# xinntao/EDVR

Hardware: AMD Instinct MI355X
Metric: EDVR-L x4 5-frame 720p clips/sec (higher is better)
Workload: dtype fp32 emulated as 2xf16 (hi+lo, 22-bit operands, 4 cross products), fp32 accumulate; 1 GPU; EDVR-L x4, 5 frames, 180x320 LR -> 720x1280, batch 10/GPU, inference; clips_per_gpu=10, global_clips=10, parallelism=clip-sharded x1, no data-path collective, world_size=1, backend=single process

## Files before the change

edvr_amd/_lib.py:

```python
import ctypes
import os

_HERE = os.path.dirname(os.path.abspath(__file__))
LIB_PATH = os.environ.get('EDVR_AMD_LIB') or os.path.join(_HERE, 'lib', 'libedvr_amd.so')

c_float_p = ctypes.c_void_p
i32, i64, f32, sz = ctypes.c_int, ctypes.c_int64, ctypes.c_float, ctypes.c_size_t
vp = ctypes.c_void_p


class ConvDesc(ctypes.Structure):
    _fields_ = [
        ('x1', vp), ('x2', vp), ('c1', i32), ('c2', i32), ('x1_img_stride', i64), ('x2_img_stride', i64),
        ('x2_div', i32), ('x2_mul', i32), ('x2_add', i32), ('n', i32), ('h', i32), ('w', i32), ('wpk', vp),
        ('bias', vp), ('co', i32), ('ks', i32), ('stride', i32), ('act', i32), ('act_from', i32), ('res1', vp),
        ('res2', vp), ('res1_img_stride', i64), ('res2_img_stride', i64), ('y', vp), ('y_img_stride', i64),
        ('out_mode', i32), ('algo', i32), ('gate', vp), ('gate_img_stride', i64), ('gate_slope', f32), ('y_scale', f32),
        ('wpk_f4', vp), ('abs_sum', vp), ('abs_sum_channels', i32), ('wpk_f4s', vp), ('x_amax', vp), ('y_amax', vp),
        ('pre', vp), ('pre_img_stride', i64), ('pre_div', i32), ('pre_mul', i32), ('pre_add', i32), ('pre_n', i32),
    ]


PROTOTYPES = {
    'edvr_version': (ctypes.c_char_p, []),
# ... 54 lines not shown
    'edvr_bd_downsample_u8': (i32, [vp, vp, i32, i32, i32, i32, i32, i32, i32, vp]),
    'edvr_bd_downsample_f32': (i32, [vp, vp, i32, i32, i32, i64, i32, i32, i32, i32, vp]),
    'edvr_imresize_bicubic_u8_windows': (i32, [vp, vp, vp, vp, i32, i32, i32, i32, i32, i32, vp]),
    'edvr_bd_downsample_u8_windows': (i32, [vp, vp, vp, vp, i32, i32, i32, i32, i32, i32, vp]),
    'edvr_adam_chunk_bytes': (sz, []),
    'edvr_adam_multi_f32': (i32, [vp, i32, ctypes.c_float, ctypes.c_float, ctypes.c_float, vp]),
    'edvr_dcnv1_fwd_ws_bytes': (sz, [i32] * 12),
    'edvr_dcnv1_fwd_f32': (i32, [vp] * 4 + [i32] * 12 + [i64, i32, vp, sz, vp]),
    'edvr_dcnv1_bwd_ws_bytes': (sz, [i32] * 12),
    'edvr_dcnv1_bwd_f32': (i32, [vp] * 7 + [i32] * 12 + [i64, i64, i32, vp, sz, vp]),
    'edvr_dcnv2_bwd_f32': (i32, [vp] * 10 + [i32] * 12 + [i64, i64, i64, i64, i32, vp, sz, vp]),
    'edvr_dcnv2_bwd_split_f32': (i32, [vp] * 10 + [i32] * 12 + [i64, i64, i64, i64, i32, vp, sz, vp, vp, vp]),
    'edvr_dcnv2_bwd_split_applies': (i32, []),
    'edvr_tsa_temporal_f32': (i32, [vp] * 5 + [i32] * 4 + [vp]),
    'edvr_tsa_temporal_pair_f32': (i32, [vp] * 5 + [i32] * 4 + [vp]),
    'edvr_pool_maxavg_3x3s2_f32': (i32, [vp, vp, i32, i32, i32, i32, vp]),
    'edvr_upsample2x_f32': (i32, [vp, vp, i32, i32, i32, f32, vp]),
    'edvr_tsa_combine_f32': (i32, [vp, vp, vp, vp, i64, vp]),
    'edvr_upsample4x_add_f32': (i32, [vp, vp, i32, i32, i32, vp]),
    'edvr_add_f32': (i32, [vp, vp, vp, i64, vp]),
    'edvr_act_bwd_f32': (i32, [vp, vp, vp, vp, vp, i32, i32, i64, i32, i32, vp]),
    'edvr_conv2d_wgrad_ws_bytes': (sz, [i32] * 7),
    'edvr_conv2d_wgrad_algo': (i32, [i32]),
    'edvr_conv2d_wgrad_kernel_name': (i32, [i32] * 8 + [ctypes.c_char_p, sz]),
    'edvr_conv2d_wgrad_f32': (i32, [vp] * 4 + [i32] * 8 + [i64, i64, i32, i32, i32, i64, i32, vp, vp, sz, vp]),
    'edvr_conv2d_wgrad_split_f32': (i32, [vp] * 4 + [i32] * 8 + [i64, i64, i32, i32, i32, i64, i32, vp, vp, sz, vp, vp, vp]),
    'edvr_conv2d_wgrad_split_applies': (i32, [i32] * 8),
    'edvr_conv2d_wgrad_split_is_direct': (i32, [i32] * 2),
    'edvr_channel_sum_f32': (i32, [vp, vp, i32, i32, i64, i64, vp, sz, vp]),
    'edvr_pixel_unshuffle2_f32': (i32, [vp, vp, i32, i32, i32, i32, vp]),
# ... 45 lines not shown
```

edvr_amd/csrc/conv1x1_s.hip:

```cpp
#include <cstdlib>

#include "common.h"
#include "pack.h"

namespace edvr {

typedef float f32x16 __attribute__((ext_vector_type(16)));
typedef int c1s_i32x4 __attribute__((ext_vector_type(4)));
typedef _Float16 c1s_f16x8 __attribute__((ext_vector_type(8)));

namespace {
__device__ __forceinline__ void c1s_split4(const float (&x)[4], float s, unsigned (&o)[4]) {
  asm volatile(
      "v_fma_mixlo_f16 %0, %4, %8, 0\n\tv_fma_mixlo_f16 %1, %5, %8, 0\n\tv_fma_mixlo_f16 %2, %6, %8, 0\n\tv_fma_mixlo_f16 %3, %7, %8, 0\n\t"
      "v_fma_mixhi_f16 %0, %4, %8, -%0 op_sel_hi:[0,0,1]\n\tv_fma_mixhi_f16 %1, %5, %8, -%1 op_sel_hi:[0,0,1]\n\t"
      "v_fma_mixhi_f16 %2, %6, %8, -%2 op_sel_hi:[0,0,1]\n\tv_fma_mixhi_f16 %3, %7, %8, -%3 op_sel_hi:[0,0,1]"
      : "=&v"(o[0]), "=&v"(o[1]), "=&v"(o[2]), "=&v"(o[3])
      : "v"(x[0]), "v"(x[1]), "v"(x[2]), "v"(x[3]), "s"(s));
}
__device__ __forceinline__ float c1s_scale(float amax) {
  const int be = (int)((__builtin_bit_cast(unsigned, amax) >> 23) & 255u);
  return __builtin_bit_cast(float, (unsigned)min(max(127 + 14 - (be - 127), 7), 215) << 23);
}
}

struct Conv1x1SArgs {
  edvr_conv2d_desc d;
  const unsigned *wq;
  int ci, cop, co_start;
  int seg_shift;
};

template <int MT>
__global__ __launch_bounds__(256, 2) void conv1x1_split_kernel(const Conv1x1SArgs a) {
  constexpr int CK = 64, MB = 32 * MT, DEPTH = 8, NW = CK * MB / 4 / 256;
  constexpr int RSRC_FLAGS = 0x00020000;
  constexpr int OOB = (int)0x80000000;
  __shared__ __attribute__((aligned(16))) unsigned wsm[2][CK * MB];
  const edvr_conv2d_desc &d = a.d;
  const float s_x = c1s_scale(__builtin_bit_cast(float, __builtin_amdgcn_readfirstlane(__builtin_bit_cast(int, *d.x_amax))));
  const float inv_sw = __builtin_bit_cast(float, __builtin_amdgcn_readfirstlane((int)a.wq[1]));
  const int tid = threadIdx.x, lane = tid & 63, half = lane >> 5, j = lane & 31;
  const int wave = __builtin_amdgcn_readfirstlane(tid >> 6);
  const int hw = d.h * d.w;
  const int img = blockIdx.z, co_blk = a.co_start + blockIdx.y * MB;
  const int p = (blockIdx.x * 4 + wave) * 32 + j;
  const bool p_ok = p < hw;

  auto uniform_ptr = [&](const float *ptr) {
    const uint64_t pv = reinterpret_cast<uint64_t>(ptr);
    return ((uint64_t)(uint32_t)__builtin_amdgcn_readfirstlane((int)(pv >> 32)) << 32) | (uint32_t)__builtin_amdgcn_readfirstlane((int)(uint32_t)pv);
  };
  const uint64_t b1 = uniform_ptr(d.x1 + (int64_t)img * d.x1_img_stride);
  uint64_t b2 = b1;
  if (d.x2) {
    const int i2 = d.x2_div > 0 ? (img / d.x2_div) * d.x2_mul + d.x2_add : img;
    b2 = uniform_ptr(d.x2 + (int64_t)i2 * d.x2_img_stride);
  }
  const int voff = p_ok ? (4 * half * hw + p) * 4 : OOB;
  const int real_steps = (d.c1 + d.c2) / 8;
  const int seg_mask = (1 << a.seg_shift) - 1;
  const int64_t plane_bytes = (int64_t)hw * 4;
  auto load_b = [&](int s, float (&v)[4]) {
    const int c = 8 * s;
    const bool first = c < d.c1;
    const int cc = first ? c : c - d.c1;
    const uint64_t base = (first ? b1 : b2) + (uint64_t)((int64_t)(cc & ~seg_mask) * plane_bytes);
    const __amdgpu_buffer_rsrc_t rs = __builtin_amdgcn_make_buffer_rsrc(reinterpret_cast<void *>(base), (short)0, 0x7fffffff, RSRC_FLAGS);
    const bool ok = s < real_steps;
#pragma unroll
    for (int i = 0; i < 4; ++i)
      v[i] = __builtin_bit_cast(float, __builtin_amdgcn_raw_buffer_load_b32(rs, ok ? voff : OOB, ok ? ((cc & seg_mask) + i) * hw * 4 : 0, 0));
  };

  const int quads_total = (d.c1 + d.c2 + 3) / 4;
  c1s_i32x4 wr[NW];
  auto w_load = [&](int c0) {
#pragma unroll
    for (int i = 0; i < NW; ++i) {
      const int e = tid + i * 256, q = e / MB, col = e - q * MB;
      const bool ok = c0 / 4 + q < quads_total;
      const c1s_i32x4 v = *reinterpret_cast<const c1s_i32x4 *>(a.wq + 16 + ((int64_t)(ok ? c0 / 4 + q : 0) * a.cop + co_blk + col) * 4);
      wr[i] = ok ? v : c1s_i32x4{0, 0, 0, 0};
    }
  };
  auto w_commit = [&](int buf) {
#pragma unroll
    for (int i = 0; i < NW; ++i) *reinterpret_cast<c1s_i32x4 *>(&wsm[buf][(tid + i * 256) * 4]) = wr[i];
  };
// ... 10 lines not shown
  w_commit(0);
  __syncthreads();

  const int chunks = a.ci / CK;
  for (int ch = 0; ch < chunks; ++ch) {
    const int buf = ch & 1;
    const bool more = ch + 1 < chunks;
    if (more) w_load((ch + 1) * CK);
    const unsigned *ws = wsm[buf] + (half * MB + j) * 4;
#pragma unroll
    for (int s = 0; s < CK / 8; ++s) {
      c1s_i32x4 av[MT];
#pragma unroll
      for (int m = 0; m < MT; ++m) av[m] = *reinterpret_cast<const c1s_i32x4 *>(ws + ((2 * s) * MB + m * 32) * 4);
      unsigned pk[4];
      c1s_split4(bq[s % DEPTH], s_x, pk);
      load_b(ch * (CK / 8) + s + DEPTH, bq[s % DEPTH]);
      c1s_i32x4 b, br;
#pragma unroll
      for (int q = 0; q < 4; ++q) {
        b[q] = (int)pk[q];
        br[q] = (int)__builtin_amdgcn_alignbit(pk[q], pk[q], 16);
      }
#pragma unroll
      for (int m = 0; m < MT; ++m) acc[m] = __builtin_amdgcn_mfma_f32_32x32x16_f16(__builtin_bit_cast(c1s_f16x8, av[m]), __builtin_bit_cast(c1s_f16x8, b), acc[m], 0, 0, 0);
#pragma unroll
      for (int m = 0; m < MT; ++m) acc[m] = __builtin_amdgcn_mfma_f32_32x32x16_f16(__builtin_bit_cast(c1s_f16x8, av[m]), __builtin_bit_cast(c1s_f16x8, br), acc[m], 0, 0, 0);
      if (s == CK / 16 && more) w_commit(buf ^ 1);
    }
    asm volatile("s_waitcnt lgkmcnt(0)\n\ts_barrier" ::: "memory");
// ... 16 lines not shown
          float v = __builtin_fmaf(acc[m][r], unscale, d.bias ? d.bias[co] : 0.f);
          if (co >= d.act_from) v = sig ? __builtin_amdgcn_rcpf(1.f + __expf(-v)) : fmaxf(v, slope * v);
          const int64_t off = (int64_t)co * hw + p;
          if (q1) v += q1[off];
          if (q2) v += q2[off];
          y[off] = v;
          vmax = max(vmax, __builtin_bit_cast(unsigned, v) & 0x7fffffffu);
        }
      }
  }
  if (d.y_amax) {
#pragma unroll
    for (int sh = 32; sh > 0; sh >>= 1) vmax = max(vmax, (unsigned)__shfl_xor((int)vmax, sh));
    if (lane == 0) atomicMax(reinterpret_cast<unsigned *>(d.y_amax), vmax);
  }
}

__global__ __launch_bounds__(1024) void conv1x1_split_scale_kernel(const float *__restrict__ w, unsigned *__restrict__ wq, int64_t total) {
  __shared__ float red[16];
  float m = 0.f;
  for (int64_t i = threadIdx.x; i < total; i += 1024) m = fmaxf(m, fabsf(w[i]));
#pragma unroll
  for (int sh = 32; sh > 0; sh >>= 1) m = fmaxf(m, __shfl_xor(m, sh));
  if ((threadIdx.x & 63) == 0) red[threadIdx.x >> 6] = m;
  __syncthreads();
  if (threadIdx.x == 0) {
    for (int i = 1; i < 16; ++i) m = fmaxf(m, red[i]);
    const unsigned field = f4s_weight_scale_field(__builtin_bit_cast(unsigned, m));
    wq[0] = field << 23;
    wq[1] = (254u - field) << 23;
// ... 43 lines not shown
  const int full = d.co / 128, rem_tiles = cdiv(d.co - full * 128, 32);
  if (full > 0) {
    a.co_start = 0;
    hipLaunchKernelGGL((conv1x1_split_kernel<4>), dim3(cdiv(hw, 128), full, d.n), dim3(256), 0, stream, a);
  }
  if (rem_tiles > 0) {
    a.co_start = full * 128;
    const dim3 grid(cdiv(hw, 128), 1, d.n);
    if (rem_tiles == 1) hipLaunchKernelGGL((conv1x1_split_kernel<1>), grid, dim3(256), 0, stream, a);
    else if (rem_tiles == 2) hipLaunchKernelGGL((conv1x1_split_kernel<2>), grid, dim3(256), 0, stream, a);
    else hipLaunchKernelGGL((conv1x1_split_kernel<3>), grid, dim3(256), 0, stream, a);
  }
  return check_launch("conv1x1_split_kernel");
}

}

extern "C" {

size_t edvr_conv2d_packed_weight_1x1s_elems(int co, int ci) {
  if (co <= 0 || ci <= 0) return 0;
  return 16 + (size_t)((ci + 63) / 64 * 16) * ((co + 127) / 128 * 128) * 4;
}

int edvr_conv2d_pack_weight_1x1s_f32(const float *w, void *wpk, int co, int ci, edvr_stream_t stream_) {
  using namespace edvr;
  EDVR_REQUIRE(w && wpk && co > 0 && ci > 0, "pack_weight_1x1s: bad arguments");
  EDVR_REQUIRE((reinterpret_cast<uintptr_t>(wpk) & 15) == 0, "pack_weight_1x1s: wpk must be 16-byte aligned");
  hipStream_t stream = as_stream(stream_);
  unsigned *wq = static_cast<unsigned *>(wpk);
  const int cop = (co + 127) / 128 * 128, quads = (ci + 63) / 64 * 16;
  hipLaunchKernelGGL(conv1x1_split_scale_kernel, dim3(1), dim3(1024), 0, stream, w, wq, (int64_t)co * ci);
  const int64_t total = (int64_t)quads * cop;
// ... 6 lines not shown
```

edvr_amd/csrc/elementwise.hip:

```cpp
#include "common.h"
#include "pixel.h"

namespace edvr {

__device__ __forceinline__ float sigmoidf(float v) { return 1.f / (1.f + __expf(-v)); }

template <int VEC, bool PAIR>
__device__ __forceinline__ void tsa_temporal_body(const float *__restrict__ emb, const float *__restrict__ emb_ref,
                                                  const float *__restrict__ aligned, float *__restrict__ out, float *__restrict__ out_rev,
                                                  float *__restrict__ prob_out, int b, int t, int c, int hw) {
  typedef float vec_t __attribute__((ext_vector_type(VEC)));
  const int hwv = hw / VEC;
  const int64_t total = (int64_t)b * t * hwv;
  for (int64_t idx = (int64_t)blockIdx.x * 256 + threadIdx.x; idx < total; idx += (int64_t)gridDim.x * 256) {
    const int pv = (int)(idx % hwv);
    const int ti = (int)((idx / hwv) % t);
    const int bi = (int)(idx / ((int64_t)hwv * t));
    const vec_t *e = reinterpret_cast<const vec_t *>(emb + ((int64_t)(bi * t + ti) * c) * hw) + pv;
    const vec_t *r = reinterpret_cast<const vec_t *>(emb_ref + ((int64_t)bi * c) * hw) + pv;
    vec_t dot = 0.f;
    for (int ch = 0; ch < c; ++ch) dot += e[(int64_t)ch * hwv] * r[(int64_t)ch * hwv];
    vec_t pr;
#pragma unroll
    for (int v = 0; v < VEC; ++v) pr[v] = sigmoidf(dot[v]);
    if (prob_out) reinterpret_cast<vec_t *>(prob_out + (int64_t)(bi * t + ti) * hw)[pv] = pr;
    const vec_t *a = reinterpret_cast<const vec_t *>(aligned + ((int64_t)(bi * t + ti) * c) * hw) + pv;
    vec_t *o = reinterpret_cast<vec_t *>(out + ((int64_t)(bi * t + ti) * c) * hw) + pv;
    if constexpr (PAIR) {
      vec_t *o2 = reinterpret_cast<vec_t *>(out_rev + ((int64_t)(bi * t + (t - 1 - ti)) * c) * hw) + pv;
      for (int ch = 0; ch < c; ++ch) {
        const vec_t m = a[(int64_t)ch * hwv] * pr;
        o[(int64_t)ch * hwv] = m;
        o2[(int64_t)ch * hwv] = m;
      }
    } else {
      for (int ch = 0; ch < c; ++ch) o[(int64_t)ch * hwv] = a[(int64_t)ch * hwv] * pr;
    }
  }
}

template <int VEC>
__global__ __launch_bounds__(256) void tsa_temporal_kernel(const float *__restrict__ emb, const float *__restrict__ emb_ref,
                                                           const float *__restrict__ aligned, float *__restrict__ out,
                                                           float *__restrict__ prob_out, int b, int t, int c, int hw) {
  tsa_temporal_body<VEC, false>(emb, emb_ref, aligned, out, nullptr, prob_out, b, t, c, hw);
}

template <int VEC>
__global__ __launch_bounds__(256) void tsa_temporal_pair_kernel(const float *__restrict__ emb, const float *__restrict__ emb_ref,
                                                                const float *__restrict__ aligned, float *__restrict__ out,
                                                                float *__restrict__ out_rev, int b, int t, int c, int hw) {
  tsa_temporal_body<VEC, true>(emb, emb_ref, aligned, out, out_rev, nullptr, b, t, c, hw);
}

__global__ __launch_bounds__(256) void pool_maxavg_kernel(const float *__restrict__ x, float *__restrict__ y, int n, int c, int h, int w,
                                                          int ho, int wo) {
  const int64_t total = (int64_t)n * c * ho * wo;
  for (int64_t idx = (int64_t)blockIdx.x * 256 + threadIdx.x; idx < total; idx += (int64_t)gridDim.x * 256) {
    const int ox = (int)(idx % wo);
    const int oy = (int)((idx / wo) % ho);
    const int ch = (int)((idx / ((int64_t)wo * ho)) % c);
    const int ni = (int)(idx / ((int64_t)wo * ho * c));
    const float *src = x + ((int64_t)ni * c + ch) * h * w;
    float mx = -INFINITY, sm = 0.f;
#pragma unroll
    for (int dy = 0; dy < 3; ++dy) {
      const int iy = oy * 2 - 1 + dy;
// ... 224 lines not shown

int edvr_tsa_temporal_f32(const float *emb, const float *emb_ref, const float *aligned, float *out, float *prob_out, int b, int t,
                          int c, int hw, edvr_stream_t stream) {
  using namespace edvr;
  EDVR_REQUIRE(emb && emb_ref && aligned && out && b > 0 && t > 0 && c > 0 && hw > 0, "tsa_temporal: bad arguments");
  if (hw % 4 == 0) {
    hipLaunchKernelGGL(tsa_temporal_kernel<4>, dim3(grid_for((int64_t)b * t * (hw / 4))), dim3(256), 0, as_stream(stream), emb, emb_ref,
                       aligned, out, prob_out, b, t, c, hw);
  } else {
    hipLaunchKernelGGL(tsa_temporal_kernel<1>, dim3(grid_for((int64_t)b * t * hw)), dim3(256), 0, as_stream(stream), emb, emb_ref,
                       aligned, out, prob_out, b, t, c, hw);
  }
  return check_launch("tsa_temporal_kernel");
}

int edvr_tsa_temporal_pair_f32(const float *emb, const float *emb_ref, const float *aligned, float *out, float *out_rev, int b, int t,
                               int c, int hw, edvr_stream_t stream) {
  using namespace edvr;
  EDVR_REQUIRE(emb && emb_ref && aligned && out && out_rev && b > 0 && t > 0 && c > 0 && hw > 0, "tsa_temporal_pair: bad arguments");
  const int64_t n = (int64_t)b * t * c * hw;
  EDVR_REQUIRE((out + n <= out_rev || out_rev + n <= out) && (out + n <= aligned || aligned + n <= out) &&
                   (out_rev + n <= aligned || aligned + n <= out_rev),
               "tsa_temporal_pair: out, out_rev and aligned must be distinct buffers");
  if (hw % 4 == 0) {
    hipLaunchKernelGGL(tsa_temporal_pair_kernel<4>, dim3(grid_for((int64_t)b * t * (hw / 4))), dim3(256), 0, as_stream(stream), emb,
                       emb_ref, aligned, out, out_rev, b, t, c, hw);
  } else {
    hipLaunchKernelGGL(tsa_temporal_pair_kernel<1>, dim3(grid_for((int64_t)b * t * hw)), dim3(256), 0, as_stream(stream), emb, emb_ref,
                       aligned, out, out_rev, b, t, c, hw);
  }
// ... 92 lines not shown
```

edvr_amd/edvr_arch.py:

```python
import torch
from torch import nn

from . import functional as F_
from .arch_util import DCNv2Pack, ResidualBlockNoBN, make_layer, warn_offset_absmean

LRELU = F_.ACT_LRELU


def _conv3(cin, cout, stride=1):
    return nn.Conv2d(cin, cout, 3, stride, 1)


class PCDAlignment(nn.Module):

    def __init__(self, num_feat=64, deformable_groups=8):
        super().__init__()
        self.offset_conv1, self.offset_conv2, self.offset_conv3 = nn.ModuleDict(), nn.ModuleDict(), nn.ModuleDict()
        self.dcn_pack, self.feat_conv = nn.ModuleDict(), nn.ModuleDict()
        for lv in (3, 2, 1):
            key = f'l{lv}'
            self.offset_conv1[key] = _conv3(2 * num_feat, num_feat)
            if lv == 3:
                self.offset_conv2[key] = _conv3(num_feat, num_feat)
            else:
# ... 47 lines not shown
        self.avg_pool = nn.AvgPool2d(3, stride=2, padding=1)
        self.spatial_attn1 = nn.Conv2d(num_frame * num_feat, num_feat, 1)
        self.spatial_attn2 = nn.Conv2d(num_feat * 2, num_feat, 1)
        self.spatial_attn3 = _conv3(num_feat, num_feat)
        self.spatial_attn4 = nn.Conv2d(num_feat, num_feat, 1)
        self.spatial_attn5 = _conv3(num_feat, num_feat)
        self.spatial_attn_l1 = nn.Conv2d(num_feat, num_feat, 1)
        self.spatial_attn_l2 = _conv3(num_feat * 2, num_feat)
        self.spatial_attn_l3 = _conv3(num_feat, num_feat)
        self.spatial_attn_add1 = nn.Conv2d(num_feat, num_feat, 1)
        self.spatial_attn_add2 = nn.Conv2d(num_feat, num_feat, 1)
        self.lrelu = nn.LeakyReLU(negative_slope=0.1, inplace=True)
        self.upsample = nn.Upsample(scale_factor=2, mode='bilinear', align_corners=False)

    def forward(self, aligned_feat):
        return self.spatial(self.temporal(aligned_feat))

    def temporal(self, aligned_feat, pair=False):
        b, t, c, h, w = aligned_feat.shape
        alias = F_.ops.carry_bound
        emb_ref = F_.conv(self.temporal_attn1, alias(aligned_feat[:, self.center_frame_idx], aligned_feat))
        emb = F_.conv(self.temporal_attn2, alias(aligned_feat.reshape(b * t, c, h, w), aligned_feat)).view(b, t, -1, h, w)
        if pair:
            mod, mod_rev = F_.tsa_temporal_pair(emb, emb_ref, aligned_feat)
            return alias(mod.view(b, t * c, h, w), mod), alias(mod_rev.view(b, t * c, h, w), mod_rev)
        mod = F_.tsa_temporal(emb, emb_ref, aligned_feat)
        return alias(mod.view(b, t * c, h, w), mod)

    def spatial(self, mod):
        feat = F_.conv(self.feat_fusion, mod, act=LRELU)
        attn = F_.conv(self.spatial_attn1, mod, act=LRELU)
        attn = F_.conv(self.spatial_attn2, F_.pool_maxavg(attn), act=LRELU)
        lvl = F_.conv(self.spatial_attn_l1, attn, act=LRELU)
        lvl = F_.conv(self.spatial_attn_l2, F_.pool_maxavg(lvl), act=LRELU)
        lvl = F_.upsample2x(F_.conv(self.spatial_attn_l3, lvl, act=LRELU))
        attn = F_.conv(self.spatial_attn3, attn, act=LRELU, res1=lvl)
        attn = F_.upsample2x(F_.conv(self.spatial_attn4, attn, act=LRELU))
        attn = F_.conv(self.spatial_attn5, attn)
        attn_add = F_.conv(self.spatial_attn_add2, F_.conv(self.spatial_attn_add1, attn, act=LRELU))
        return F_.tsa_combine(feat, attn, attn_add)


class PredeblurModule(nn.Module):

    def __init__(self, num_in_ch=3, num_feat=64, hr_in=False):
        super().__init__()
# ... 107 lines not shown
            f1 = F_.conv(self.conv_1x1, self.predeblur(frames), out=head)
        else:
            f1 = F_.conv(self.conv_first, frames, act=LRELU, out=head)
        if out is None:
            f1 = self.feature_extraction(f1)
        else:
            for i, blk in enumerate(blocks):
                f1 = blk(f1, out=o1 if i == len(blocks) - 1 else None)
        f2 = F_.conv(self.conv_l2_2, F_.conv(self.conv_l2_1, f1, act=LRELU), act=LRELU, out=o2)
        f3 = F_.conv(self.conv_l3_2, F_.conv(self.conv_l3_1, f2, act=LRELU), act=LRELU, out=o3)
        return [f1, f2, f3]

    def restore_from_features(self, pyr, x_center, b, t, out_dtype=torch.float32, out=None, keep=None, elem=None, accumulate='only', scale=1.0,
                              acc=None, bands=None):
        self._check_tail_args(out_dtype, out, keep, elem, accumulate, scale, acc, bands)
        operand, sink = self.align_windows(pyr, b, t)
        return self._restore_aligned(operand, x_center, b, t, out_dtype, out, keep, elem, accumulate, scale, acc, bands, sink)

    def align_windows(self, pyr, b, t, pair=False):
        f1, f2, f3 = pyr
        ctr = self.center_frame_idx
        h, w = f1.shape[2], f1.shape[3]
        if pair and 2 * ctr != t - 1:
            raise ValueError(f'align_windows(pair=True): the reversed clip keeps its centre only when it is the middle frame, got {ctr} of {t}')
        sink = []
        dcns = self.pcd_align.dcn_modules()
        for m in dcns:
            m.stats_sink = sink
        try:
            aligned = self.pcd_align.align([f1, f2, f3], [f1, f2, f3], ref_map=(t, t, ctr))
        finally:
            for m in dcns:
                m.stats_sink = None
        flat = aligned
        aligned = F_.ops.carry_bound(aligned.view(b, t, -1, h, w), aligned)
        if self.taps is not None:
            self.taps['aligned'] = aligned
        if self.with_tsa:
            operand = self.fusion.temporal(aligned, pair=pair)
            return (*operand, sink) if pair else (operand, sink)
        operand = F_.ops.carry_bound(aligned.view(b, -1, h, w), aligned)
        if not pair:
            return operand, sink
        if torch.is_grad_enabled():
            raise RuntimeError('align_windows(pair=True) has no backward: call it under torch.no_grad()')
        table = torch.arange(b * t, dtype=torch.int32, device=flat.device).view(b, t).flip(1).reshape(-1)
        rev = F_.ops.gather_images([flat], table)[0]
        return operand, F_.ops.carry_bound(rev.view(b, -1, h, w), rev), sink

    def restore_from_aligned(self, operand, x_center, b, t, out_dtype=torch.float32, out=None, keep=None, elem=None, accumulate='only', scale=1.0,
                             acc=None, bands=None, sink=None):
        self._check_tail_args(out_dtype, out, keep, elem, accumulate, scale, acc, bands)
        return self._restore_aligned(operand, x_center, b, t, out_dtype, out, keep, elem, accumulate, scale, acc, bands, sink)
# ... 4 lines not shown
            raise ValueError(f'out_dtype must be torch.float32 or torch.uint8, got {out_dtype}')
        if out_dtype == torch.uint8 and torch.is_grad_enabled():
            raise RuntimeError('the uint8 output of EDVR.restore_from_features has no backward: call it under torch.no_grad()')
        if out is None and keep is not None:
            raise ValueError('keep= names a rectangle of the result to store into out=: it needs out')
        if out is not None and torch.is_grad_enabled():
            raise RuntimeError('EDVR.restore_from_features(out=) writes in place and has no backward: call it under torch.no_grad()')
        if elem is None and (accumulate != 'only' or scale != 1.0 or (acc is not None and bands is None)):
            raise ValueError('accumulate=, scale= and acc= belong to a self-ensemble element: they need elem')
        if (elem is not None or bands is not None) and (out is None or (out_dtype == torch.uint8) != (acc is not None)):
            raise ValueError('elem= and bands= store into out= (and, with uint8 output, accumulate in acc=)')

    def _restore_aligned(self, operand, x_center, b, t, out_dtype, out, keep, elem, accumulate, scale, acc, bands, sink):
        dst = out
        taps = self.taps
        feat = self.fusion.spatial(operand) if self.with_tsa else F_.conv(self.fusion, operand)
        if taps is not None:
            taps['fused'] = feat
        out = self.reconstruction(feat)
        if taps is not None:
            taps['trunk'] = out
        out = F_.conv(self.upconv1, out, act=LRELU, out_mode=F_.OUT_PIXEL_SHUFFLE2)
        out = F_.conv(self.upconv2, out, act=LRELU, out_mode=F_.OUT_PIXEL_SHUFFLE2)
        out = F_.conv(self.conv_hr, out, act=LRELU)
        if dst is not None:
            ky, kx = keep if keep is not None else (0, 0)
            if bands is not None:
                how = dict(bands=bands, elem=0 if elem is None else elem, mode=accumulate, scale=scale)
                if self.hr_in:
                    last = F_.conv(self.conv_last, out, res1=x_center)
                    out = (F_.ops.f32_to_u8_hwc_rect_blend(last, dst, acc, ky, kx, **how) if acc is not None
# ... 15 lines not shown
                tail = F_.ops.f32_to_u8_hwc_rect if out_dtype == torch.uint8 else F_.ops.copy_rect
                out = tail(F_.conv(self.conv_last, out, res1=x_center), dst, ky, kx)
            else:
                tail = F_.ops.upsample4x_add_u8_rect if out_dtype == torch.uint8 else F_.ops.upsample4x_add_rect
                out = tail(F_.conv(self.conv_last, out), x_center, dst, ky, kx)
        elif self.hr_in:
            out = F_.conv(self.conv_last, out, res1=x_center)
            if out_dtype == torch.uint8:
                out = F_.ops.f32_to_u8_hwc(out)
        elif out_dtype == torch.uint8:
            out = F_.ops.upsample4x_add_u8(F_.conv(self.conv_last, out), x_center)
        else:
            out = F_.upsample4x_add(F_.conv(self.conv_last, out), x_center)
        if sink:
            self._queue_offset_check(sink, b, t)
        F_.ops.split_guard_submit(operand.device)
        return out

    def _queue_offset_check(self, sink, b, t):
        if not sink:
            return
        import torch
        sums = torch.stack([e[0] for e in sink]).view(len(sink), 2, b, t).sum(2)
        recs = [(per_img * b, module) for _, per_img, module in sink]
        if torch.cuda.is_current_stream_capturing():
            self._captured_offset_stats = (sums, recs)
            return
        if torch.is_grad_enabled() and F_.ops.HINT_WAIT:
            self._examine_offsets(sums.cpu(), recs)
            return
        host = torch.empty(sums.shape, dtype=sums.dtype, pin_memory=True)
# ... 27 lines not shown
```

edvr_amd/functional.py:

```python
import math
import os

import torch

from . import ops
from .ops import ACT_LRELU, ACT_NONE, ACT_RELU, ACT_SIGMOID, OUT_NCHW, OUT_PIXEL_SHUFFLE2


def _conv_geometry(m):
    ks, st = m.kernel_size, m.stride
    if (ks[0] != ks[1] or ks[0] not in (1, 3) or st[0] != st[1] or st[0] not in (1, 2) or (ks[0] == 1 and st[0] != 1)
            or tuple(m.padding) != (ks[0] // 2, ks[0] // 2) or tuple(m.dilation) != (1, 1) or m.groups != 1):
        raise NotImplementedError(
            f'edvr_amd conv kernel supports 3x3 (stride 1/2, pad 1) and 1x1 convolutions, dilation 1, groups 1; got {m}')
    return ks[0], st[0]


def _needs_grad(*ts):
    return torch.is_grad_enabled() and any(t is not None and t.requires_grad for t in ts)


def conv(m, x, *, x2=None, x2_map=None, act=ACT_NONE, act_from=0, res1=None, res2=None, out_mode=OUT_NCHW, y_scale=1.0,
         abs_sum_channels=0, ci_range=None, use_bias=True, pre=None, pre_map=None, out=None):
    ks, stride = _conv_geometry(m)
# ... 141 lines not shown


def tsa_temporal(emb, emb_ref, aligned):
    if _needs_grad(emb, emb_ref, aligned):
        from . import autograd as ag
        return ag.TsaTemporal.apply(emb, emb_ref, aligned)
    return ops.tsa_temporal(emb, emb_ref, aligned)


def tsa_temporal_pair(emb, emb_ref, aligned):
    if torch.is_grad_enabled():
        raise RuntimeError('tsa_temporal_pair has no backward: call it under torch.no_grad()')
    return ops.tsa_temporal_pair(emb, emb_ref, aligned)


def tsa_combine(feat, attn, attn_add):
    if _needs_grad(feat, attn, attn_add):
        from . import autograd as ag
        return ag.TsaCombine.apply(feat, attn, attn_add)
    return ops.tsa_combine(feat, attn, attn_add)


def add(a, b):
    if _needs_grad(a, b):
        from . import autograd as ag
        return ag.Add.apply(a, b)
    return ops.add(a, b)


def upsample4x_add(y, base):
# ... 5 lines not shown
```

edvr_amd/ops.py:

```python
import ctypes
import os
import weakref

import torch

from . import _lib
from ._lib import (ACT_LRELU, ACT_NONE, ACT_RELU, ACT_SIGMOID, CONV_AUTO, CONV_DIRECT, CONV_WINOGRAD, CONV_WINOGRAD_F4, CONV_WINOGRAD_F4S, OUT_NCHW,
                   OUT_PIXEL_SHUFFLE2)


def _stream():
    return ctypes.c_void_p(torch.cuda.current_stream().cuda_stream)


def _ptr(t):
    return ctypes.c_void_p(t.data_ptr()) if t is not None else ctypes.c_void_p(0)


def require_gpu(*tensors, dtypes=(torch.float32,)):
    seen = None
    for t in tensors:
        if t is None:
            continue
        if not t.is_cuda:
# ... 262 lines not shown
        self.buf, self.i, self.mark, self.retired = None, 0, 0, []

    def fresh(self, device):
        if self.buf is not None and self.i > self.mark:
            self.retired.append(self.buf[self.mark:self.i])
        self.buf, self.i, self.mark = torch.zeros(self.BLOCK, dtype=torch.float32, device=device), 0, 0

    def slot(self, device):
        if self.buf is None or self.i >= self.buf.numel():
            if self.buf is not None and device.type == 'cuda' and torch.cuda.is_current_stream_capturing():
                raise RuntimeError('edvr_amd: the magnitude-bound arena ran out of slots inside a hipGraph capture (more than '
                                   f'{self.BLOCK} split-operand launches in one captured region); capture a smaller region')
            self.fresh(device)
        self.i += 1
        return self.buf[self.i - 1:self.i]

    def take_unexamined(self):
        out, self.retired = self.retired, []
        if self.buf is not None and self.i > self.mark:
            out.append(self.buf[self.mark:self.i])
            self.mark = self.i
        return out


_AMAX_ARENAS = {}


def _arena(device):
    key = (device.index, torch.cuda.current_stream(device).cuda_stream)
    a = _AMAX_ARENAS.get(key)
# ... 448 lines not shown

def tsa_temporal(emb, emb_ref, aligned, want_prob=False):
    require_gpu(emb, emb_ref, aligned)
    b, t, c, h, w = aligned.shape
    al_in = aligned
    emb, emb_ref, aligned = emb.contiguous(), emb_ref.contiguous(), aligned.contiguous()
    out = torch.empty_like(aligned)
    prob = torch.empty(b, t, h, w, dtype=torch.float32, device=aligned.device) if want_prob else None
    _run('tsa_temporal', lambda: _lib.check(_lib.lib().edvr_tsa_temporal_f32(_ptr(emb), _ptr(emb_ref), _ptr(aligned), _ptr(out), _ptr(prob), b, t, c, h * w,
                                                _stream()),
                                       'edvr_tsa_temporal_f32'), 0, _nb(emb, emb_ref, aligned, out, prob))
    carry_bound(out, al_in)
    return (out, prob) if want_prob else out


def tsa_temporal_pair(emb, emb_ref, aligned, out=None, out_rev=None):
    if torch.is_grad_enabled():
        raise RuntimeError('tsa_temporal_pair has no backward: call it under torch.no_grad()')
    require_gpu(emb, emb_ref, aligned, out, out_rev)
    b, t, c, h, w = aligned.shape
    al_in = aligned
    emb, emb_ref, aligned = emb.contiguous(), emb_ref.contiguous(), aligned.contiguous()
    if tuple(emb.shape) != (b, t, c, h, w) or tuple(emb_ref.shape) != (b, c, h, w):
        raise ValueError(f'tsa_temporal_pair: emb {tuple(emb.shape)} / emb_ref {tuple(emb_ref.shape)} do not match aligned {tuple(aligned.shape)}')
    out = torch.empty_like(aligned) if out is None else out
    out_rev = torch.empty_like(aligned) if out_rev is None else out_rev
    nbytes = 4 * aligned.numel()
    for o in (out, out_rev):
        if tuple(o.shape) != (b, t, c, h, w) or not o.is_contiguous():
            raise ValueError(f'tsa_temporal_pair: outputs are contiguous {(b, t, c, h, w)} tensors, got {tuple(o.shape)} / strides {o.stride()}')
# ... 823 lines not shown
```

include/edvr_amd.h:

```cpp
#ifndef EDVR_AMD_H
#define EDVR_AMD_H

#include <stddef.h>
#include <stdint.h>

#ifdef __cplusplus
extern "C" {
#endif

#define EDVR_OK 0
#define EDVR_ERR_ARG (-1)
#define EDVR_ERR_UNSUPPORTED (-2)
#define EDVR_ERR_LAUNCH (-3)
#define EDVR_ERR_WORKSPACE (-4)

typedef void *edvr_stream_t;

const char *edvr_version(void);
const char *edvr_last_error(void);
int edvr_check_device(void);

#define EDVR_ACT_NONE 0
#define EDVR_ACT_RELU 1
#define EDVR_ACT_LRELU 2
// ... 120 lines not shown
                               int groups, int dg);
int edvr_dcnv1_fwd_f32(const float *x, const float *offset, const float *weight, float *y, int B, int C, int H, int W,
                       int Co, int kh, int kw, int stride, int pad, int dil, int groups, int dg, int64_t offset_bstride,
                       int halo_hint, void *ws, size_t ws_bytes, edvr_stream_t stream);
size_t edvr_dcnv1_bwd_ws_bytes(int B, int C, int H, int W, int Co, int kh, int kw, int stride, int pad, int dil,
                               int groups, int dg);
int edvr_dcnv1_bwd_f32(const float *x, const float *offset, const float *weight, const float *dy, float *dx,
                       float *doffset, float *dweight, int B, int C, int H, int W, int Co, int kh, int kw, int stride,
                       int pad, int dil, int groups, int dg, int64_t offset_bstride, int64_t doffset_bstride,
                       int scatter_hint, void *ws, size_t ws_bytes, edvr_stream_t stream);

int edvr_tsa_temporal_f32(const float *emb, const float *emb_ref, const float *aligned, float *out, float *prob_out,
                          int b, int t, int c, int hw, edvr_stream_t stream);
int edvr_tsa_temporal_pair_f32(const float *emb, const float *emb_ref, const float *aligned, float *out, float *out_rev,
                               int b, int t, int c, int hw, edvr_stream_t stream);
int edvr_pool_maxavg_3x3s2_f32(const float *x, float *y, int n, int c, int h, int w, edvr_stream_t stream);
int edvr_upsample2x_f32(const float *x, float *y, int nc, int h, int w, float scale, edvr_stream_t stream);
int edvr_tsa_combine_f32(const float *feat, const float *attn, const float *attn_add, float *y, int64_t numel,
                         edvr_stream_t stream);
int edvr_upsample4x_add_f32(const float *base, float *y, int nc, int h, int w, edvr_stream_t stream);
int edvr_add_f32(const float *a, const float *b, float *y, int64_t numel, edvr_stream_t stream);
int edvr_act_bwd_f32(const float *dy, const float *y, const float *res1, const float *res2, float *dz, int n, int c,
                     int64_t hw, int act, int act_from, edvr_stream_t stream);
int edvr_abs_sum_f32(const float *x, float *out, int n, int64_t per_img, int64_t img_stride, edvr_stream_t stream);
int edvr_abs_stats_f32(const float *x, float *out, int n, int64_t per_img, int w, int64_t img_stride, edvr_stream_t stream);

size_t edvr_conv2d_wgrad_ws_bytes(int n, int ci, int h, int w, int co, int ks, int stride);
int edvr_conv2d_wgrad_f32(const float *x1, const float *x2, const float *dz, float *dw, int c1, int c2, int n, int h, int w,
                          int co, int ks, int stride, int64_t x1_img_stride, int64_t x2_img_stride, int x2_div, int x2_mul,
                          int x2_add, int64_t dz_img_stride, int accumulate, float *dbias, void *ws, size_t ws_bytes,
// ... 118 lines not shown
```

Before: 100.3 clips/s.

## Fuse TSA temporal attention weighting into paired feat_fusion/spatial_attn1 1x1 convs

Adds a fused TSA front path for inference. A new kernel computes only the per-frame sigmoid attention probabilities, without writing the modulated aligned features. A paired split-f16 1x1 conv kernel then scales each input channel by its frame probability while loading, and computes both feat_fusion and spatial_attn1 in one launch, interleaving blocks between the two weight sets. This removes the write and re-read of the t*c modulated tensor and one conv launch. In exchange the conv inner loop gains a per-step multiply and a prob load at frame boundaries, and the path is inference-only behind an environment switch.

```diff
diff --git a/edvr_amd/_lib.py b/edvr_amd/_lib.py
--- a/edvr_amd/_lib.py
+++ b/edvr_amd/_lib.py
@@ -92,6 +92,9 @@
     'edvr_dcnv2_bwd_split_applies': (i32, []),
     'edvr_tsa_temporal_f32': (i32, [vp] * 5 + [i32] * 4 + [vp]),
     'edvr_tsa_temporal_pair_f32': (i32, [vp] * 5 + [i32] * 4 + [vp]),
+    'edvr_tsa_temporal_prob_f32': (i32, [vp] * 3 + [i32] * 4 + [vp]),
+    'edvr_tsa_fused_front_supported': (i32, [i32] * 6),
+    'edvr_tsa_fused_front_f32': (i32, [vp] * 9 + [i32] * 7 + [vp]),
     'edvr_pool_maxavg_3x3s2_f32': (i32, [vp, vp, i32, i32, i32, i32, vp]),
     'edvr_upsample2x_f32': (i32, [vp, vp, i32, i32, i32, f32, vp]),
     'edvr_tsa_combine_f32': (i32, [vp, vp, vp, vp, i64, vp]),
diff --git a/edvr_amd/csrc/conv1x1_s.hip b/edvr_amd/csrc/conv1x1_s.hip
--- a/edvr_amd/csrc/conv1x1_s.hip
+++ b/edvr_amd/csrc/conv1x1_s.hip
@@ -31,8 +31,13 @@
   int seg_shift;
 };
 
-template <int MT>
-__global__ __launch_bounds__(256, 2) void conv1x1_split_kernel(const Conv1x1SArgs a) {
+struct Conv1x1STsa {
+  const float *prob;
+  int t, steps_per_frame;
+};
+
+template <int MT, bool TSA>
+__device__ __forceinline__ void conv1x1_split_body(const Conv1x1SArgs &a, const Conv1x1STsa &ts, const int tile, const int co_tile, const int img) {
   constexpr int CK = 64, MB = 32 * MT, DEPTH = 8, NW = CK * MB / 4 / 256;
   constexpr int RSRC_FLAGS = 0x00020000;
   constexpr int OOB = (int)0x80000000;
@@ -43,8 +48,8 @@
   const int tid = threadIdx.x, lane = tid & 63, half = lane >> 5, j = lane & 31;
   const int wave = __builtin_amdgcn_readfirstlane(tid >> 6);
   const int hw = d.h * d.w;
-  const int img = blockIdx.z, co_blk = a.co_start + blockIdx.y * MB;
-  const int p = (blockIdx.x * 4 + wave) * 32 + j;
+  const int co_blk = a.co_start + co_tile * MB;
+  const int p = (tile * 4 + wave) * 32 + j;
   const bool p_ok = p < hw;
 
   auto uniform_ptr = [&](const float *ptr) {
@@ -73,6 +78,19 @@
       v[i] = __builtin_bit_cast(float, __builtin_amdgcn_raw_buffer_load_b32(rs, ok ? voff : OOB, ok ? ((cc & seg_mask) + i) * hw * 4 : 0, 0));
   };
 
+  float pr = 0.f, pr_next = 0.f;
+  int frame_next = 1, step_switch = ts.steps_per_frame;
+  auto load_prob = [&](int f) {
+    const uint64_t pb = uniform_ptr(ts.prob + (int64_t)img * ts.t * hw);
+    const __amdgpu_buffer_rsrc_t rs = __builtin_amdgcn_make_buffer_rsrc(reinterpret_cast<void *>(pb), (short)0, 0x7fffffff, RSRC_FLAGS);
+    const bool ok = f < ts.t;
+    return __builtin_bit_cast(float, __builtin_amdgcn_raw_buffer_load_b32(rs, (ok && p_ok) ? p * 4 : OOB, ok ? f * hw * 4 : 0, 0));
+  };
+  if constexpr (TSA) {
+    pr = load_prob(0);
+    pr_next = load_prob(1);
+  }
+
   const int quads_total = (d.c1 + d.c2 + 3) / 4;
   c1s_i32x4 wr[NW];
   auto w_load = [&](int c0) {
@@ -113,6 +131,15 @@
 #pragma unroll
       for (int m = 0; m < MT; ++m) av[m] = *reinterpret_cast<const c1s_i32x4 *>(ws + ((2 * s) * MB + m * 32) * 4);
       unsigned pk[4];
+      if constexpr (TSA) {
+        if (ch * (CK / 8) + s == step_switch) {
+          pr = pr_next;
+          step_switch += ts.steps_per_frame;
+          pr_next = load_prob(++frame_next);
+        }
+#pragma unroll
+        for (int i = 0; i < 4; ++i) bq[s % DEPTH][i] *= pr;
+      }
       c1s_split4(bq[s % DEPTH], s_x, pk);
       load_b(ch * (CK / 8) + s + DEPTH, bq[s % DEPTH]);
       c1s_i32x4 b, br;
@@ -159,6 +186,34 @@
     for (int sh = 32; sh > 0; sh >>= 1) vmax = max(vmax, (unsigned)__shfl_xor((int)vmax, sh));
     if (lane == 0) atomicMax(reinterpret_cast<unsigned *>(d.y_amax), vmax);
   }
+}
+
+template <int MT>
+__global__ __launch_bounds__(256, 2) void conv1x1_split_kernel(const Conv1x1SArgs a) {
+  conv1x1_split_body<MT, false>(a, Conv1x1STsa{}, blockIdx.x, blockIdx.y, blockIdx.z);
+}
+
+struct Conv1x1SPair {
+  const unsigned *wq;
+  const float *bias;
+  float *y, *y_amax;
+};
+
+template <int MT>
+__global__ __launch_bounds__(256, 2) void conv1x1_split_tsa_kernel(const Conv1x1SArgs a0, const Conv1x1STsa ts, const Conv1x1SPair second,
+                                                                   const int tiles, const int items) {
+  const int L = blockIdx.x, k = L >> 3;
+  const int item = (k >> 1) * 8 + (L & 7);
+  if (item >= items) return;
+  Conv1x1SArgs a = a0;
+  if (k & 1) {
+    a.wq = second.wq;
+    a.d.bias = second.bias;
+    a.d.y = second.y;
+    a.d.y_amax = second.y_amax;
+  }
+  const int img = item / tiles;
+  conv1x1_split_body<MT, true>(a, ts, item - img * tiles, 0, img);
 }
 
 __global__ __launch_bounds__(1024) void conv1x1_split_scale_kernel(const float *__restrict__ w, unsigned *__restrict__ wq, int64_t total) {
@@ -232,9 +287,70 @@
   return check_launch("conv1x1_split_kernel");
 }
 
+static edvr_conv2d_desc tsa_front_desc(int b, int t, int c, int h, int w, int co) {
+  edvr_conv2d_desc d = {};
+  d.n = b, d.c1 = t * c, d.h = h, d.w = w, d.co = co, d.ks = 1, d.stride = 1, d.out_mode = EDVR_OUT_NCHW, d.algo = EDVR_CONV_AUTO;
+  d.x1_img_stride = (int64_t)t * c * h * w, d.y_img_stride = (int64_t)co * h * w;
+  return d;
+}
+
+static bool tsa_front_eligible(const edvr_conv2d_desc &d0, int t, int c) {
+  static const bool on = []() {
+    const char *e = getenv("EDVR_TSA_FUSED");
+    return !(e && e[0] == '0');
+  }();
+  if (!on || t <= 0 || c <= 0 || (c & 7) || d0.n <= 0 || d0.h <= 0 || d0.w <= 0 || d0.co > 128) return false;
+  edvr_conv2d_desc d = d0;
+  d.wpk_f4s = d.x_amax = reinterpret_cast<const float *>(&d);
+  if (!conv1x1_split_eligible(d)) return false;
+  const int64_t hw = (int64_t)d.h * d.w;
+  return (int64_t)t * hw * 4 < ((int64_t)1 << 31) && (int64_t)d.n * cdiv((int)hw, 128) < ((int64_t)1 << 26);
+}
+
 }
 
 extern "C" {
+
+int edvr_tsa_fused_front_supported(int b, int t, int c, int h, int w, int co) {
+  using namespace edvr;
+  if (b <= 0 || t <= 0 || c <= 0 || h <= 0 || w <= 0 || co <= 0 || (int64_t)h * w >= ((int64_t)1 << 28)) return 0;
+  return tsa_front_eligible(tsa_front_desc(b, t, c, h, w, co), t, c) ? 1 : 0;
+}
+
+int edvr_tsa_fused_front_f32(const float *aligned, const float *prob, const void *wpk_pair, const float *bias_a, const float *bias_b, float *y_a,
+                             float *y_b, const float *x_amax, float *y_amax, int b, int t, int c, int h, int w, int co, int act,
+                             edvr_stream_t stream_) {
+  using namespace edvr;
+  EDVR_REQUIRE(aligned && prob && wpk_pair && y_a && y_b && x_amax, "tsa_fused_front: null pointer");
+  EDVR_REQUIRE((reinterpret_cast<uintptr_t>(wpk_pair) & 15) == 0, "tsa_fused_front: packed weights must be 16-byte aligned");
+  if (edvr_tsa_fused_front_supported(b, t, c, h, w, co) != 1) {
+    set_error("tsa_fused_front: shape b=%d t=%d c=%d h=%d w=%d co=%d is not eligible (ask edvr_tsa_fused_front_supported)", b, t, c, h, w, co);
+    return EDVR_ERR_UNSUPPORTED;
+  }
+  Conv1x1SArgs a;
+  a.d = tsa_front_desc(b, t, c, h, w, co);
+  a.d.x1 = aligned, a.d.bias = bias_a, a.d.y = y_a, a.d.x_amax = x_amax, a.d.y_amax = y_amax, a.d.act = act;
+  a.wq = static_cast<const unsigned *>(wpk_pair);
+  a.ci = ((t * c + 63) / 64) * 64;
+  a.cop = 128;
+  a.co_start = 0;
+  const int hw = h * w;
+  a.seg_shift = 30;
+  while (((int64_t)1 << a.seg_shift) * hw * 4 >= ((int64_t)1 << 31)) --a.seg_shift;
+  if (a.seg_shift < 3) a.seg_shift = 3;
+  const Conv1x1STsa ts = {prob, t, c / 8};
+  const Conv1x1SPair second = {a.wq + edvr_conv2d_packed_weight_1x1s_elems(co, t * c), bias_b, y_b, y_amax ? y_amax + 1 : nullptr};
+  const int tiles = cdiv(hw, 128), items = tiles * b;
+  const dim3 grid((unsigned)(cdiv(items, 8) * 16));
+  hipStream_t stream = as_stream(stream_);
+  switch (cdiv(co, 32)) {
+    case 1: hipLaunchKernelGGL((conv1x1_split_tsa_kernel<1>), grid, dim3(256), 0, stream, a, ts, second, tiles, items); break;
+    case 2: hipLaunchKernelGGL((conv1x1_split_tsa_kernel<2>), grid, dim3(256), 0, stream, a, ts, second, tiles, items); break;
+    case 3: hipLaunchKernelGGL((conv1x1_split_tsa_kernel<3>), grid, dim3(256), 0, stream, a, ts, second, tiles, items); break;
+    default: hipLaunchKernelGGL((conv1x1_split_tsa_kernel<4>), grid, dim3(256), 0, stream, a, ts, second, tiles, items); break;
+  }
+  return check_launch("conv1x1_split_tsa_kernel");
+}
 
 size_t edvr_conv2d_packed_weight_1x1s_elems(int co, int ci) {
   if (co <= 0 || ci <= 0) return 0;
diff --git a/edvr_amd/csrc/elementwise.hip b/edvr_amd/csrc/elementwise.hip
--- a/edvr_amd/csrc/elementwise.hip
+++ b/edvr_amd/csrc/elementwise.hip
@@ -5,7 +5,7 @@
 
 __device__ __forceinline__ float sigmoidf(float v) { return 1.f / (1.f + __expf(-v)); }
 
-template <int VEC, bool PAIR>
+template <int VEC, bool PAIR, bool PROB_ONLY = false>
 __device__ __forceinline__ void tsa_temporal_body(const float *__restrict__ emb, const float *__restrict__ emb_ref,
                                                   const float *__restrict__ aligned, float *__restrict__ out, float *__restrict__ out_rev,
                                                   float *__restrict__ prob_out, int b, int t, int c, int hw) {
@@ -23,7 +23,8 @@
     vec_t pr;
 #pragma unroll
     for (int v = 0; v < VEC; ++v) pr[v] = sigmoidf(dot[v]);
-    if (prob_out) reinterpret_cast<vec_t *>(prob_out + (int64_t)(bi * t + ti) * hw)[pv] = pr;
+    if (PROB_ONLY || prob_out) reinterpret_cast<vec_t *>(prob_out + (int64_t)(bi * t + ti) * hw)[pv] = pr;
+    if constexpr (PROB_ONLY) continue;
     const vec_t *a = reinterpret_cast<const vec_t *>(aligned + ((int64_t)(bi * t + ti) * c) * hw) + pv;
     vec_t *o = reinterpret_cast<vec_t *>(out + ((int64_t)(bi * t + ti) * c) * hw) + pv;
     if constexpr (PAIR) {
@@ -51,6 +52,12 @@
                                                                 const float *__restrict__ aligned, float *__restrict__ out,
                                                                 float *__restrict__ out_rev, int b, int t, int c, int hw) {
   tsa_temporal_body<VEC, true>(emb, emb_ref, aligned, out, out_rev, nullptr, b, t, c, hw);
+}
+
+template <int VEC>
+__global__ __launch_bounds__(256) void tsa_temporal_prob_kernel(const float *__restrict__ emb, const float *__restrict__ emb_ref,
+                                                                float *__restrict__ prob_out, int b, int t, int c, int hw) {
+  tsa_temporal_body<VEC, false, true>(emb, emb_ref, nullptr, nullptr, nullptr, prob_out, b, t, c, hw);
 }
 
 __global__ __launch_bounds__(256) void pool_maxavg_kernel(const float *__restrict__ x, float *__restrict__ y, int n, int c, int h, int w,
@@ -305,6 +312,19 @@
   return check_launch("tsa_temporal_kernel");
 }
 
+int edvr_tsa_temporal_prob_f32(const float *emb, const float *emb_ref, float *prob_out, int b, int t, int c, int hw, edvr_stream_t stream) {
+  using namespace edvr;
+  EDVR_REQUIRE(emb && emb_ref && prob_out && b > 0 && t > 0 && c > 0 && hw > 0, "tsa_temporal_prob: bad arguments");
+  if (hw % 4 == 0) {
+    hipLaunchKernelGGL(tsa_temporal_prob_kernel<4>, dim3(grid_for((int64_t)b * t * (hw / 4))), dim3(256), 0, as_stream(stream), emb, emb_ref,
+                       prob_out, b, t, c, hw);
+  } else {
+    hipLaunchKernelGGL(tsa_temporal_prob_kernel<1>, dim3(grid_for((int64_t)b * t * hw)), dim3(256), 0, as_stream(stream), emb, emb_ref,
+                       prob_out, b, t, c, hw);
+  }
+  return check_launch("tsa_temporal_prob_kernel");
+}
+
 int edvr_tsa_temporal_pair_f32(const float *emb, const float *emb_ref, const float *aligned, float *out, float *out_rev, int b, int t,
                                int c, int hw, edvr_stream_t stream) {
   using namespace edvr;
diff --git a/edvr_amd/edvr_arch.py b/edvr_amd/edvr_arch.py
--- a/edvr_amd/edvr_arch.py
+++ b/edvr_amd/edvr_arch.py
@@ -85,13 +85,28 @@
         self.upsample = nn.Upsample(scale_factor=2, mode='bilinear', align_corners=False)
 
     def forward(self, aligned_feat):
+        if self.fused_front_applies(aligned_feat):
+            return self.tail(*self.front(aligned_feat))
         return self.spatial(self.temporal(aligned_feat))
 
-    def temporal(self, aligned_feat, pair=False):
+    def _embeddings(self, aligned_feat):
         b, t, c, h, w = aligned_feat.shape
         alias = F_.ops.carry_bound
         emb_ref = F_.conv(self.temporal_attn1, alias(aligned_feat[:, self.center_frame_idx], aligned_feat))
         emb = F_.conv(self.temporal_attn2, alias(aligned_feat.reshape(b * t, c, h, w), aligned_feat)).view(b, t, -1, h, w)
+        return emb, emb_ref
+
+    def fused_front_applies(self, aligned_feat):
+        return F_.tsa_fused_front_applies(aligned_feat, self.feat_fusion, self.spatial_attn1)
+
+    def front(self, aligned_feat):
+        emb, emb_ref = self._embeddings(aligned_feat)
+        return F_.tsa_fused_front(emb, emb_ref, aligned_feat, self.feat_fusion, self.spatial_attn1)
+
+    def temporal(self, aligned_feat, pair=False):
+        b, t, c, h, w = aligned_feat.shape
+        alias = F_.ops.carry_bound
+        emb, emb_ref = self._embeddings(aligned_feat)
         if pair:
             mod, mod_rev = F_.tsa_temporal_pair(emb, emb_ref, aligned_feat)
             return alias(mod.view(b, t * c, h, w), mod), alias(mod_rev.view(b, t * c, h, w), mod_rev)
@@ -99,8 +114,9 @@
         return alias(mod.view(b, t * c, h, w), mod)
 
     def spatial(self, mod):
-        feat = F_.conv(self.feat_fusion, mod, act=LRELU)
-        attn = F_.conv(self.spatial_attn1, mod, act=LRELU)
+        return self.tail(F_.conv(self.feat_fusion, mod, act=LRELU), F_.conv(self.spatial_attn1, mod, act=LRELU))
+
+    def tail(self, feat, attn):
         attn = F_.conv(self.spatial_attn2, F_.pool_maxavg(attn), act=LRELU)
         lvl = F_.conv(self.spatial_attn_l1, attn, act=LRELU)
         lvl = F_.conv(self.spatial_attn_l2, F_.pool_maxavg(lvl), act=LRELU)
@@ -238,10 +254,10 @@
     def restore_from_features(self, pyr, x_center, b, t, out_dtype=torch.float32, out=None, keep=None, elem=None, accumulate='only', scale=1.0,
                               acc=None, bands=None):
         self._check_tail_args(out_dtype, out, keep, elem, accumulate, scale, acc, bands)
-        operand, sink = self.align_windows(pyr, b, t)
+        operand, sink = self.align_windows(pyr, b, t, _fuse_front=True)
         return self._restore_aligned(operand, x_center, b, t, out_dtype, out, keep, elem, accumulate, scale, acc, bands, sink)
 
-    def align_windows(self, pyr, b, t, pair=False):
+    def align_windows(self, pyr, b, t, pair=False, _fuse_front=False):
         f1, f2, f3 = pyr
         ctr = self.center_frame_idx
         h, w = f1.shape[2], f1.shape[3]
@@ -261,6 +277,8 @@
         if self.taps is not None:
             self.taps['aligned'] = aligned
         if self.with_tsa:
+            if _fuse_front and not pair and self.taps is None and self.fusion.fused_front_applies(aligned):
+                return self.fusion.front(aligned), sink
             operand = self.fusion.temporal(aligned, pair=pair)
             return (*operand, sink) if pair else (operand, sink)
         operand = F_.ops.carry_bound(aligned.view(b, -1, h, w), aligned)
@@ -295,7 +313,10 @@
     def _restore_aligned(self, operand, x_center, b, t, out_dtype, out, keep, elem, accumulate, scale, acc, bands, sink):
         dst = out
         taps = self.taps
-        feat = self.fusion.spatial(operand) if self.with_tsa else F_.conv(self.fusion, operand)
+        if self.with_tsa:
+            feat = self.fusion.tail(*operand) if isinstance(operand, tuple) else self.fusion.spatial(operand)
+        else:
+            feat = F_.conv(self.fusion, operand)
         if taps is not None:
             taps['fused'] = feat
         out = self.reconstruction(feat)
@@ -341,7 +362,7 @@
             out = F_.upsample4x_add(F_.conv(self.conv_last, out), x_center)
         if sink:
             self._queue_offset_check(sink, b, t)
-        F_.ops.split_guard_submit(operand.device)
+        F_.ops.split_guard_submit(x_center.device)
         return out
 
     def _queue_offset_check(self, sink, b, t):
diff --git a/edvr_amd/functional.py b/edvr_amd/functional.py
--- a/edvr_amd/functional.py
+++ b/edvr_amd/functional.py
@@ -179,6 +179,14 @@
     return ops.tsa_temporal_pair(emb, emb_ref, aligned)
 
 
+def tsa_fused_front_applies(aligned, feat_fusion, spatial_attn1):
+    return not torch.is_grad_enabled() and ops.tsa_fused_front_supported(aligned, feat_fusion, spatial_attn1)
+
+
+def tsa_fused_front(emb, emb_ref, aligned, feat_fusion, spatial_attn1):
+    return ops.tsa_fused_front(emb, emb_ref, aligned, feat_fusion, spatial_attn1, act=ACT_LRELU)
+
+
 def tsa_combine(feat, attn, attn_add):
     if _needs_grad(feat, attn, attn_add):
         from . import autograd as ag
diff --git a/edvr_amd/ops.py b/edvr_amd/ops.py
--- a/edvr_amd/ops.py
+++ b/edvr_amd/ops.py
@@ -300,6 +300,14 @@
             self.fresh(device)
         self.i += 1
         return self.buf[self.i - 1:self.i]
+
+    def slots(self, device, n):
+        if self.buf is not None and self.i + n > self.buf.numel():
+            self.i = self.buf.numel()
+        first = self.slot(device)
+        for _ in range(n - 1):
+            self.slot(device)
+        return self.buf[self.i - n:self.i] if n > 1 else first
 
     def take_unexamined(self):
         out, self.retired = self.retired, []
@@ -778,6 +786,86 @@
     return (out, prob) if want_prob else out
 
 
+TSA_FUSED = os.environ.get('EDVR_TSA_FUSED', '1') != '0'
+
+
+def tsa_temporal_prob(emb, emb_ref, out=None):
+    require_gpu(emb, emb_ref, out)
+    b, t, c, h, w = emb.shape
+    emb, emb_ref = emb.contiguous(), emb_ref.contiguous()
+    if tuple(emb_ref.shape) != (b, c, h, w):
+        raise ValueError(f'tsa_temporal_prob: emb_ref {tuple(emb_ref.shape)} does not match emb {tuple(emb.shape)}')
+    if out is None:
+        out = torch.empty(b, t, h, w, dtype=torch.float32, device=emb.device)
+    elif tuple(out.shape) != (b, t, h, w) or not out.is_contiguous():
+        raise ValueError(f'tsa_temporal_prob: out is a contiguous {(b, t, h, w)} tensor, got {tuple(out.shape)} / strides {out.stride()}')
+    _run('tsa_temporal_prob_kernel', lambda: _lib.check(_lib.lib().edvr_tsa_temporal_prob_f32(_ptr(emb), _ptr(emb_ref), _ptr(out), b, t, c, h * w, _stream()),
+                                                   'edvr_tsa_temporal_prob_f32'), 0, _nb(emb, emb_ref, out))
+    return out
+
+
+def tsa_fused_front_supported(aligned, conv_a, conv_b):
+    if not (TSA_FUSED and F4S_INFERENCE and CONV_ALGO != CONV_DIRECT and aligned.is_cuda and aligned.dtype == torch.float32 and aligned.dim() == 5):
+        return False
+    b, t, c, h, w = aligned.shape
+    wa, wb = conv_a.weight, conv_b.weight
+    if tuple(wa.shape) != (wa.shape[0], t * c, 1, 1) or wb.shape != wa.shape or not (wa.is_cuda and wb.is_cuda):
+        return False
+    return bool(_lib.lib().edvr_tsa_fused_front_supported(b, t, c, h, w, wa.shape[0]))
+
+
+def pack_tsa_front_weights(wa, wb):
+    require_gpu(wa, wb)
+    key, wid = ('tsa_front',), id(wa)
+    ent = _PACKED.get(wid)
+    if ent is not None and ent[0]() is wa:
+        hit = ent[1].get(key)
+        if hit is not None and hit[0] == wa._version and hit[2] == wa.data_ptr() and hit[3]() is wb and hit[4:] == (wb._version, wb.data_ptr()):
+            return hit[1]
+    else:
+        ent = (weakref.ref(wa, lambda _r, wid=wid: _PACKED.pop(wid, None)), {})
+        _PACKED[wid] = ent
+    L = _lib.lib()
+    co, ci = wa.shape[0], wa.shape[1]
+    n_el = L.edvr_conv2d_packed_weight_1x1s_elems(co, ci)
+    out = torch.empty(2 * n_el, dtype=torch.int32, device=wa.device)
+    for i, w in enumerate((wa, wb)):
+        _lib.check(L.edvr_conv2d_pack_weight_1x1s_f32(_ptr(w.detach().contiguous()), _ptr(out[i * n_el:]), co, ci, _stream()), 'edvr_conv2d_pack_weight_1x1s_f32')
+    ent[1][key] = (wa._version, out, wa.data_ptr(), weakref.ref(wb), wb._version, wb.data_ptr())
+    return out
+
+
+def tsa_fused_front(emb, emb_ref, aligned, conv_a, conv_b, act=ACT_LRELU):
+    if torch.is_grad_enabled():
+        raise RuntimeError('tsa_fused_front has no backward: call it under torch.no_grad()')
+    require_gpu(emb, emb_ref, aligned, conv_a.weight, conv_b.weight)
+    if not tsa_fused_front_supported(aligned, conv_a, conv_b):
+        raise RuntimeError(f'tsa_fused_front: not eligible for aligned {tuple(aligned.shape)} (ask tsa_fused_front_supported)')
+    b, t, c, h, w = aligned.shape
+    al_in, aligned = aligned, aligned.contiguous()
+    if tuple(emb.shape) != (b, t, c, h, w) or tuple(emb_ref.shape) != (b, c, h, w):
+        raise ValueError(f'tsa_fused_front: emb {tuple(emb.shape)} / emb_ref {tuple(emb_ref.shape)} do not match aligned {tuple(aligned.shape)}')
+    dev, co = aligned.device, conv_a.weight.shape[0]
+    prob = workspace(4 * b * t * h * w, dev, tag='tsa_prob')[:4 * b * t * h * w].view(torch.float32).view(b, t, h, w)
+    tsa_temporal_prob(emb, emb_ref, out=prob)
+    wpk = pack_tsa_front_weights(conv_a.weight, conv_b.weight)
+    x_amax = input_bound(al_in, aligned.view(b, t * c, h, w))
+    ya = torch.empty(b, co, h, w, dtype=torch.float32, device=dev)
+    yb = torch.empty(b, co, h, w, dtype=torch.float32, device=dev)
+    y_bounds = _arena(dev).slots(dev, 2)
+    bias_a = conv_a.bias.detach() if conv_a.bias is not None else None
+    bias_b = conv_b.bias.detach() if conv_b.bias is not None else None
+    flops = 2.0 * (2 * co) * t * c * b * h * w
+    nbytes = 4.0 * (aligned.numel() + prob.numel() + ya.numel() + yb.numel() + 2 * co * t * c)
+    _run('conv1x1_split_kernel[tsa]',
+         lambda: _lib.check(_lib.lib().edvr_tsa_fused_front_f32(_ptr(aligned), _ptr(prob), _ptr(wpk), _ptr(bias_a), _ptr(bias_b), _ptr(ya), _ptr(yb), _ptr(x_amax),
+                                                                 _ptr(y_bounds), b, t, c, h, w, co, act, _stream()), 'edvr_tsa_fused_front_f32'),
+         flops, nbytes, 4.0 * flops)
+    set_bound(ya, y_bounds[0:1])
+    set_bound(yb, y_bounds[1:2])
+    return ya, yb
+
+
 def tsa_temporal_pair(emb, emb_ref, aligned, out=None, out_rev=None):
     if torch.is_grad_enabled():
         raise RuntimeError('tsa_temporal_pair has no backward: call it under torch.no_grad()')
diff --git a/include/edvr_amd.h b/include/edvr_amd.h
--- a/include/edvr_amd.h
+++ b/include/edvr_amd.h
@@ -158,6 +158,12 @@
                           int b, int t, int c, int hw, edvr_stream_t stream);
 int edvr_tsa_temporal_pair_f32(const float *emb, const float *emb_ref, const float *aligned, float *out, float *out_rev,
                                int b, int t, int c, int hw, edvr_stream_t stream);
+int edvr_tsa_temporal_prob_f32(const float *emb, const float *emb_ref, float *prob_out, int b, int t, int c, int hw,
+                               edvr_stream_t stream);
+int edvr_tsa_fused_front_supported(int b, int t, int c, int h, int w, int co);
+int edvr_tsa_fused_front_f32(const float *aligned, const float *prob, const void *wpk_pair, const float *bias_a, const float *bias_b,
+                             float *y_a, float *y_b, const float *x_amax, float *y_amax, int b, int t, int c, int h, int w, int co,
+                             int act, edvr_stream_t stream);
 int edvr_pool_maxavg_3x3s2_f32(const float *x, float *y, int n, int c, int h, int w, edvr_stream_t stream);
 int edvr_upsample2x_f32(const float *x, float *y, int nc, int h, int w, float scale, edvr_stream_t stream);
 int edvr_tsa_combine_f32(const float *feat, const float *attn, const float *attn_add, float *y, int64_t numel,
```

New measurement: 100.5 clips/s (median of 6 runs). About the same (+0.2%).
